# sutro-sh/sutro

Measured on AMD Instinct MI355X. Metric: output_tokens_per_sec, higher is better.
Workload: dtype bf16; 1 GPU; model=qwen-3-32b, global_batch=2048, seq_len=256, parallelism=dp1, prompt_len=128, priming=seeded

## Files before the change

### csrc/bindings.cpp

```cpp
#include <torch/extension.h>

#include <hip/hip_runtime.h>
#include <c10/hip/HIPStream.h>

#define CHECK_CUDA(x) TORCH_CHECK((x).is_cuda(), #x " must be a GPU tensor")
#define CHECK_CONTIG(x) TORCH_CHECK((x).is_contiguous(), #x " must be contiguous")
#define CHECK_BF16(x) \
  TORCH_CHECK((x).scalar_type() == at::kBFloat16, #x " must be bf16")

static hipStream_t cur_stream() {
  return c10::hip::getCurrentHIPStream().stream();
}

extern "C" {
void sutro_rmsnorm(void*, const void*, const void*, float, long, int,
                   hipStream_t);
void sutro_fused_add_rmsnorm(void*, void*, const void*, float, long, int,
                             hipStream_t);
void sutro_silu_mul(void*, const void*, long, int, hipStream_t);
void sutro_rope_and_cache(void*, void*, const void*, const long*, const long*,
                          void*, void*, const float*, int, int, int, int, int,
                          hipStream_t);
static bool is_fp8(const torch::Tensor& t) {
  return t.scalar_type() == at::kFloat8_e4m3fn;
}
void sutro_mean_pool_normalize(float*, const void*, const int*, int, int,
                               hipStream_t);
void sutro_attn_decode(void*, const void*, const void*, const void*,
                       const int*, const int*, int, int, int, int, int, int,
                       int, float, hipStream_t);
void sutro_attn_prefill(void*, const void*, const void*, const void*,
                        const int*, const int*, const int*, const int*,
                        const int*, int, int, int, int, int, int, float,
                        hipStream_t);
void sutro_mfma32_probe(float*, const void*, const void*, hipStream_t);
void sutro_gemm_tn_launch(void*, const void*, const void*, const void*, int,
                          int, long, int, int, int, int, hipStream_t);
void sutro_mfma16_probe(float*, const void*, const void*, hipStream_t);
void sutro_hd64_stage_probe(float*, float*, void*, const void*, const void*,
                            const void*, int, float, hipStream_t);
void sutro_qkv_prep(const void*, void*, void*, void*, const long*, const long*,
                    const float*, const void*, const void*, float, int, int,
                    int, int, int, int, int, hipStream_t);
void sutro_sampler_fused(const void*, int, const float*, const float*,
                         const int*, const float*, const unsigned int*, int,
                         long, int, int, int*, float*, hipStream_t);
void sutro_grouped_gemm(void*, const void*, const void*, const int*,
                        const int*, const int*, int, int, int, long, int,
                        int, hipStream_t);
void sutro_moe_combine(void*, const void*, const long*, const float*, int,
                       int, int, hipStream_t);
void sutro_logit_penalties(void*, int, const int*, const int*, const int*,
                           const int*, const int*, const float*, const float*,
                           const float*, const int*, const float*, int, int,
                           long, int, int, int, int, int, hipStream_t);
void sutro_quant_rows_fp8(void*, float*, const void*, const int*, int, long,
                          int, int, hipStream_t);
void sutro_grouped_gemm_fp8(void*, const void*, const float*, const void*,
                            const float*, const int*, const int*, const int*,
                            int, int, int, long, int, int, hipStream_t);
void sutro_quant_weight_mxfp4(void*, void*, const void*, long, int, int,
                              hipStream_t);
void sutro_grouped_gemm_mxfp4(void*, const void*, const float*, const void*,
                              const void*, const int*, const int*, const int*,
                              int, int, int, long, int, int, hipStream_t);
}

void rmsnorm(torch::Tensor out, torch::Tensor x, torch::Tensor w, double eps) {
  CHECK_CUDA(x); CHECK_CONTIG(x); CHECK_BF16(x);
  const long C = x.size(-1);
  const long rows = x.numel() / C;
  TORCH_CHECK(C % 8 == 0 && C <= 16384, "unsupported row size ", C);
  sutro_rmsnorm(out.data_ptr(), x.data_ptr(), w.data_ptr(), (float)eps, rows,
                (int)C, cur_stream());
}

void fused_add_rmsnorm(torch::Tensor x, torch::Tensor residual, torch::Tensor w,
                       double eps) {
  CHECK_CUDA(x); CHECK_CONTIG(x); CHECK_BF16(x); CHECK_CONTIG(residual);
  const long C = x.size(-1);
  const long rows = x.numel() / C;
  TORCH_CHECK(C % 8 == 0 && C <= 16384, "unsupported row size ", C);
  sutro_fused_add_rmsnorm(x.data_ptr(), residual.data_ptr(), w.data_ptr(),
                          (float)eps, rows, (int)C, cur_stream());
}

void silu_mul(torch::Tensor out, torch::Tensor x) {
  CHECK_CUDA(x); CHECK_CONTIG(x); CHECK_BF16(x);
  const long I = x.size(-1) / 2;
  const long T = x.numel() / (2 * I);
  TORCH_CHECK(I % 8 == 0, "intermediate size must be a multiple of 8");
  sutro_silu_mul(out.data_ptr(), x.data_ptr(), T, (int)I, cur_stream());
}

void rope_and_cache(torch::Tensor q, torch::Tensor k, torch::Tensor v,
                    torch::Tensor positions, torch::Tensor slot_mapping,
                    torch::Tensor k_cache, torch::Tensor v_cache,
                    torch::Tensor cos_sin) {
  CHECK_CUDA(q); CHECK_CONTIG(q); CHECK_BF16(q);
  CHECK_CONTIG(k); CHECK_CONTIG(v); CHECK_CONTIG(k_cache);
  TORCH_CHECK(cos_sin.scalar_type() == at::kFloat, "cos_sin must be f32");
  const int T = q.size(0), Hq = q.size(1), D = q.size(2);
  const int Hk = k.size(1);
  const int bs = k_cache.size(2);
  TORCH_CHECK(D % 2 == 0 && D / 2 <= 128, "unsupported head_dim ", D);
  sutro_rope_and_cache(q.data_ptr(), k.data_ptr(), v.data_ptr(),
                       positions.data_ptr<long>(), slot_mapping.data_ptr<long>(),
                       k_cache.data_ptr(), v_cache.data_ptr(),
                       cos_sin.data_ptr<float>(), T, Hq, Hk, D, bs,
                       cur_stream());
}

void mean_pool_normalize(torch::Tensor out, torch::Tensor hidden,
                         torch::Tensor qlocs) {
  CHECK_CUDA(hidden); CHECK_CONTIG(hidden); CHECK_BF16(hidden);
  const int S = out.size(0), H = hidden.size(-1);
  TORCH_CHECK(H % 8 == 0, "hidden size must be a multiple of 8");
  sutro_mean_pool_normalize(out.data_ptr<float>(), hidden.data_ptr(),
                            qlocs.data_ptr<int>(), S, H, cur_stream());
}

void paged_attention(torch::Tensor out, torch::Tensor q, torch::Tensor k_cache,
                     torch::Tensor v_cache, torch::Tensor block_tables,
                     torch::Tensor seq_lens, torch::Tensor qlocs, double scale,
                     int64_t num_decodes, torch::Tensor tile_seq,
                     torch::Tensor tile_q0, int64_t prefill_token_count) {
  CHECK_CUDA(q); CHECK_CONTIG(q); CHECK_BF16(q); CHECK_CONTIG(k_cache);
  const int Hq = q.size(1), D = q.size(2);
  const int Hk = k_cache.size(1);
  const int bs = k_cache.size(2);
  const int S = seq_lens.size(0);
  TORCH_CHECK(D == 128 || D == 64,
              "attention kernels support head_dim 64/128 (got ", D, ")");
  TORCH_CHECK(bs == 32, "attention kernels require kv_block_size 32");
  TORCH_CHECK(Hq % Hk == 0 && Hq / Hk <= 8,
              "GQA group size must divide and be <= 8");
  const int bt_stride = block_tables.size(1);
  const int n_tiles = tile_seq.numel();
  if (n_tiles > 0) {
    sutro_attn_prefill(out.data_ptr(), q.data_ptr(), k_cache.data_ptr(),
                       v_cache.data_ptr(), block_tables.data_ptr<int>(),
                       seq_lens.data_ptr<int>(), qlocs.data_ptr<int>(),
                       tile_seq.data_ptr<int>(), tile_q0.data_ptr<int>(),
                       n_tiles, bt_stride, Hq, Hk, D,
                       is_fp8(k_cache) ? 1 : 0, (float)scale, cur_stream());
  }
  if (num_decodes > 0) {
    const long dec_off = prefill_token_count;
    const int seq_offset = S - (int)num_decodes;
    const u_int16_t* qp = (const u_int16_t*)q.data_ptr();
    u_int16_t* op = (u_int16_t*)out.data_ptr();
    sutro_attn_decode(op + dec_off * Hq * D, qp + dec_off * Hq * D,
                      k_cache.data_ptr(), v_cache.data_ptr(),
                      block_tables.data_ptr<int>(), seq_lens.data_ptr<int>(),
                      bt_stride, (int)num_decodes, Hq, Hk, D,
                      is_fp8(k_cache) ? 1 : 0, seq_offset, (float)scale,
                      cur_stream());
  }
}

void qkv_prep(torch::Tensor qkv, torch::Tensor q_out, torch::Tensor k_cache,
              torch::Tensor v_cache, torch::Tensor positions,
              torch::Tensor slot_mapping, torch::Tensor cos_sin,
              c10::optional<torch::Tensor> q_norm_w,
              c10::optional<torch::Tensor> k_norm_w, double eps) {
  CHECK_CUDA(qkv); CHECK_CONTIG(qkv); CHECK_BF16(qkv);
  CHECK_CONTIG(q_out); CHECK_CONTIG(k_cache); CHECK_CONTIG(v_cache);
  const int T = qkv.size(0);
  const int Hq = q_out.size(1), D = q_out.size(2);
  const int Hk = k_cache.size(1);
  const int bs = k_cache.size(2);
  const int row_stride = qkv.size(1);
  TORCH_CHECK(row_stride == Hq * D + 2 * Hk * D, "qkv width mismatch");
  const void* qw = q_norm_w ? q_norm_w->data_ptr() : nullptr;
  const void* kw = k_norm_w ? k_norm_w->data_ptr() : nullptr;
  sutro_qkv_prep(qkv.data_ptr(), q_out.data_ptr(), k_cache.data_ptr(),
                 v_cache.data_ptr(), positions.data_ptr<long>(),
                 slot_mapping.data_ptr<long>(), cos_sin.data_ptr<float>(), qw,
                 kw, (float)eps, T, Hq, Hk, D, bs, row_stride,
                 is_fp8(k_cache) ? 1 : 0, cur_stream());
}

torch::Tensor gemm_tn(torch::Tensor x, torch::Tensor w,
                      c10::optional<torch::Tensor> res, long bm, long bn,
                      long swz, long xcd_swz) {
  CHECK_CUDA(x); CHECK_BF16(x); CHECK_CUDA(w); CHECK_BF16(w);
  TORCH_CHECK(x.is_contiguous() && w.is_contiguous(), "contiguous required");
  const long M = x.size(0), K = x.size(1), N = w.size(0);
  TORCH_CHECK(w.size(1) == K, "K mismatch");
  TORCH_CHECK(M % bm == 0 && K % 64 == 0, "shape not tile-divisible");
  auto out = torch::empty({M, N}, x.options());
  const void* rp = nullptr;
  if (res.has_value()) {
    CHECK_CUDA(*res); CHECK_BF16(*res);
    TORCH_CHECK(res->is_contiguous() && res->size(0) == M && res->size(1) == N,
                "res shape");
    rp = res->data_ptr();
  }
  sutro_gemm_tn_launch(out.data_ptr(), x.data_ptr(), w.data_ptr(), rp, (int)M,
                       (int)N, K, (int)bm, (int)bn, (int)swz, (int)xcd_swz,
                       cur_stream());
  return out;
}

torch::Tensor mfma32_probe(torch::Tensor a, torch::Tensor b) {
  CHECK_CUDA(a); CHECK_BF16(a);
  auto c = torch::zeros({32, 32}, a.options().dtype(at::kFloat));
  sutro_mfma32_probe(c.data_ptr<float>(), a.data_ptr(), b.data_ptr(),
                     cur_stream());
  return c;
}

std::vector<torch::Tensor> hd64_stage_probe(torch::Tensor q, torch::Tensor k,
                                             torch::Tensor v, long L,
                                             double scale) {
  CHECK_CUDA(q); CHECK_BF16(q);
  auto fopt = q.options().dtype(at::kFloat);
  auto vt = torch::zeros({64 * 40}, fopt);
  auto p = torch::zeros({16 * 40}, fopt);
  auto out = torch::zeros({1, 64}, q.options());
  sutro_hd64_stage_probe(vt.data_ptr<float>(), p.data_ptr<float>(),
                         out.data_ptr(), q.data_ptr(), k.data_ptr(),
                         v.data_ptr(), (int)L, (float)scale, cur_stream());
  return {vt, p, out};
}

torch::Tensor mfma16_probe(torch::Tensor a, torch::Tensor b) {
  CHECK_CUDA(a); CHECK_BF16(a);
  auto c = torch::zeros({16, 16}, a.options().dtype(at::kFloat));
  sutro_mfma16_probe(c.data_ptr<float>(), a.data_ptr(), b.data_ptr(),
                     cur_stream());
  return c;
}

void grouped_gemm(torch::Tensor out, torch::Tensor a, torch::Tensor w,
                  c10::optional<torch::Tensor> row_tok, torch::Tensor tile_off,
                  torch::Tensor counts, long max_tiles, bool gate_silu,
                  long bm) {
  TORCH_CHECK(bm == 64 || bm == 128, "bm must be 64 or 128");
  CHECK_CUDA(a); CHECK_CONTIG(a); CHECK_BF16(a);
  CHECK_CUDA(w); CHECK_CONTIG(w); CHECK_BF16(w);
  CHECK_CONTIG(out); CHECK_BF16(out);
  const long E = w.size(0), N = w.size(1), K = w.size(2);
  const long n_cols = gate_silu ? N / 2 : N;
  TORCH_CHECK(K % 64 == 0 && n_cols % 64 == 0,
              "grouped_gemm needs K, n_cols multiples of 64 (K=", K,
              ", n_cols=", n_cols, ")");
  TORCH_CHECK(a.size(1) == K, "A K mismatch");
  TORCH_CHECK(out.size(1) == n_cols, "out width mismatch");
  TORCH_CHECK(tile_off.scalar_type() == at::kInt
              && counts.scalar_type() == at::kInt, "tile_off/counts int32");
  TORCH_CHECK(tile_off.numel() == E + 1 && counts.numel() == E, "seg sizes");
  const int* rt = nullptr;
  if (row_tok.has_value()) {
    TORCH_CHECK(row_tok->scalar_type() == at::kInt, "row_tok int32");
    rt = row_tok->data_ptr<int>();
  }
  sutro_grouped_gemm(out.data_ptr(), a.data_ptr(), w.data_ptr(), rt,
                     tile_off.data_ptr<int>(), counts.data_ptr<int>(), (int)E,
                     (int)max_tiles, (int)n_cols, K, gate_silu ? 1 : 0,
                     (int)bm, cur_stream());
}

void quant_rows_fp8(torch::Tensor x, torch::Tensor out_q,
                    torch::Tensor out_scale,
                    c10::optional<torch::Tensor> row_limit, long limit_mul) {
  CHECK_CUDA(x); CHECK_CONTIG(x); CHECK_BF16(x);
  CHECK_CUDA(out_q); CHECK_CONTIG(out_q);
  CHECK_CUDA(out_scale); CHECK_CONTIG(out_scale);
  TORCH_CHECK(x.dim() == 2 && out_q.dim() == 2, "x, out_q must be 2-D");
  TORCH_CHECK(is_fp8(out_q), "out_q must be float8_e4m3fn");
  TORCH_CHECK(out_scale.scalar_type() == at::kFloat, "out_scale must be f32");
  const long R = x.size(0), K = x.size(1), Kp = out_q.size(1);
  TORCH_CHECK(K % 8 == 0 && K > 0, "K must be a positive multiple of 8");
  TORCH_CHECK(Kp == (K + 127) / 128 * 128, "out_q width must be K rounded "
              "up to 128 (K=", K, ", Kp=", Kp, ")");
  TORCH_CHECK(Kp < (1L << 31), "row too wide");
  TORCH_CHECK(out_q.size(0) >= R && out_scale.numel() >= R,
              "out_q/out_scale hold fewer rows than x");
  const int* lim = nullptr;
  if (row_limit.has_value()) {
    CHECK_CUDA(*row_limit);
    TORCH_CHECK(row_limit->scalar_type() == at::kInt
                && row_limit->numel() >= 1, "row_limit int32 scalar");
    lim = row_limit->data_ptr<int>();
  }
  sutro_quant_rows_fp8(out_q.data_ptr(), out_scale.data_ptr<float>(),
                       x.data_ptr(), lim, (int)limit_mul, R, (int)K, (int)Kp,
                       cur_stream());
}

void grouped_gemm_fp8(torch::Tensor out, torch::Tensor a_q,
                      torch::Tensor a_scale, torch::Tensor w_q,
                      torch::Tensor w_scale,
                      c10::optional<torch::Tensor> row_tok,
                      torch::Tensor tile_off, torch::Tensor counts,
                      long max_tiles, bool gate_silu, long bm) {
  TORCH_CHECK(bm == 64 || bm == 128, "bm must be 64 or 128");
  CHECK_CUDA(a_q); CHECK_CONTIG(a_q); CHECK_CUDA(w_q); CHECK_CONTIG(w_q);
  TORCH_CHECK(is_fp8(a_q) && is_fp8(w_q), "a_q, w_q must be float8_e4m3fn");
  CHECK_CUDA(a_scale); CHECK_CONTIG(a_scale);
  CHECK_CUDA(w_scale); CHECK_CONTIG(w_scale);
  TORCH_CHECK(a_scale.scalar_type() == at::kFloat
              && w_scale.scalar_type() == at::kFloat, "scales must be f32");
  CHECK_CUDA(out); CHECK_CONTIG(out); CHECK_BF16(out);
  TORCH_CHECK(w_q.dim() == 3 && a_q.dim() == 2 && out.dim() == 2, "ranks");
  const long E = w_q.size(0), N = w_q.size(1), Kp = w_q.size(2);
  const long n_cols = gate_silu ? N / 2 : N;
  TORCH_CHECK(Kp % 128 == 0 && Kp > 0 && n_cols % 64 == 0 && n_cols > 0,
              "grouped_gemm_fp8 needs Kp a multiple of 128 and n_cols of 64 "
              "(Kp=", Kp, ", n_cols=", n_cols, ")");
  TORCH_CHECK(a_q.size(1) == Kp, "A Kp mismatch");
  TORCH_CHECK(out.size(1) == n_cols, "out width mismatch");
  TORCH_CHECK(max_tiles >= 0 && out.size(0) >= max_tiles * bm,
              "out holds fewer rows than max_tiles * bm");
  TORCH_CHECK(w_scale.numel() == E * N, "w_scale must be [E, N]");
  TORCH_CHECK(tile_off.scalar_type() == at::kInt
              && counts.scalar_type() == at::kInt, "tile_off/counts int32");
  TORCH_CHECK(tile_off.numel() == E + 1 && counts.numel() == E, "seg sizes");
  const int* rt = nullptr;
  if (row_tok.has_value()) {
    TORCH_CHECK(row_tok->scalar_type() == at::kInt, "row_tok int32");
    TORCH_CHECK(row_tok->numel() >= max_tiles * bm, "row_tok too short");
    rt = row_tok->data_ptr<int>();
  } else {
    TORCH_CHECK(a_q.size(0) >= max_tiles * bm,
                "a_q holds fewer rows than max_tiles * bm");
  }
  TORCH_CHECK(!gate_silu || rt, "the gate/up stage gathers through row_tok");
  TORCH_CHECK(a_scale.numel() >= a_q.size(0), "a_scale shorter than a_q");
  sutro_grouped_gemm_fp8(out.data_ptr(), a_q.data_ptr(),
                         a_scale.data_ptr<float>(), w_q.data_ptr(),
                         w_scale.data_ptr<float>(), rt,
                         tile_off.data_ptr<int>(), counts.data_ptr<int>(),
                         (int)E, (int)max_tiles, (int)n_cols, Kp,
                         gate_silu ? 1 : 0, (int)bm, cur_stream());
}

void quant_weight_mxfp4(torch::Tensor x, torch::Tensor out_q,
                        torch::Tensor out_scale) {
  CHECK_CUDA(x); CHECK_CONTIG(x); CHECK_BF16(x);
  CHECK_CUDA(out_q); CHECK_CONTIG(out_q);
  CHECK_CUDA(out_scale); CHECK_CONTIG(out_scale);
  TORCH_CHECK(x.dim() == 2 && out_q.dim() == 2 && out_scale.dim() == 2,
              "x, out_q, out_scale must be 2-D");
  TORCH_CHECK(out_q.scalar_type() == at::kByte
              && out_scale.scalar_type() == at::kByte,
              "out_q, out_scale must be uint8");
  const long R = x.size(0), K = x.size(1);
  TORCH_CHECK(K % 8 == 0 && K > 0, "K must be a positive multiple of 8");
  const long Kp = (K + 127) / 128 * 128;
  TORCH_CHECK(Kp < (1L << 31), "row too wide");
  TORCH_CHECK(out_q.size(1) == Kp / 2 && out_scale.size(1) == Kp / 32,
              "out_q / out_scale widths must be Kp/2 and Kp/32 with Kp = K "
// ... 50 lines not shown
  TORCH_CHECK(a_scale.numel() >= a_q.size(0), "a_scale shorter than a_q");
  sutro_grouped_gemm_mxfp4(out.data_ptr(), a_q.data_ptr(),
                           a_scale.data_ptr<float>(), w_q.data_ptr(),
                           w_scale.data_ptr(), rt,
                           tile_off.data_ptr<int>(), counts.data_ptr<int>(),
                           (int)E, (int)max_tiles, (int)n_cols, Kp,
                           gate_silu ? 1 : 0, (int)bm, cur_stream());
}

void moe_combine(torch::Tensor out, torch::Tensor rows, torch::Tensor padpos,
                 torch::Tensor w) {
  CHECK_CUDA(rows); CHECK_CONTIG(rows); CHECK_BF16(rows);
  CHECK_CONTIG(out); CHECK_BF16(out);
  const long T = out.size(0), h = out.size(1), k = padpos.size(1);
  TORCH_CHECK(h % 8 == 0, "h must be a multiple of 8");
  TORCH_CHECK(padpos.scalar_type() == at::kLong, "padpos must be int64");
  TORCH_CHECK(w.scalar_type() == at::kFloat, "w must be f32");
  TORCH_CHECK(padpos.is_contiguous() && w.is_contiguous(), "contig");
  sutro_moe_combine(out.data_ptr(), rows.data_ptr(),
                    padpos.data_ptr<long>(), w.data_ptr<float>(), (int)T,
                    (int)h, (int)k, cur_stream());
}

void sampler_fused(torch::Tensor logits, torch::Tensor temps,
                   torch::Tensor topps, torch::Tensor topks, torch::Tensor us,
                   c10::optional<torch::Tensor> mask, long vl,
                   torch::Tensor out_tok, torch::Tensor out_lp) {
  CHECK_CUDA(logits); CHECK_CONTIG(logits);
  const bool f32 = logits.scalar_type() == at::kFloat;
  TORCH_CHECK(f32 || logits.scalar_type() == at::kBFloat16,
              "logits must be bf16 or f32");
  const long n = logits.size(0), v_row = logits.size(1);
  TORCH_CHECK(vl <= v_row, "vocab_limit exceeds logits row");
  TORCH_CHECK(temps.numel() >= n && topps.numel() >= n && topks.numel() >= n
              && us.numel() >= n, "param tensors too small");
  TORCH_CHECK(topks.scalar_type() == at::kInt, "topks must be int32");
  const unsigned int* mptr = nullptr;
  int w_words = 0;
  if (mask.has_value()) {
    auto& mt = mask.value();
    CHECK_CUDA(mt); CHECK_CONTIG(mt);
    TORCH_CHECK(mt.scalar_type() == at::kInt, "mask must be int32 packed");
    TORCH_CHECK(mt.size(0) == n, "mask rows mismatch");
    w_words = (int)mt.size(1);
    TORCH_CHECK((long)w_words * 32 >= vl, "mask too narrow for vocab_limit");
    mptr = (const unsigned int*)mt.data_ptr();
  }
  sutro_sampler_fused(logits.data_ptr(), f32 ? 1 : 0,
                      temps.data_ptr<float>(), topps.data_ptr<float>(),
                      topks.data_ptr<int>(), us.data_ptr<float>(), mptr,
                      (int)n, v_row, (int)vl, w_words,
                      out_tok.data_ptr<int>(), out_lp.data_ptr<float>(),
                      cur_stream());
}

void logit_penalties(torch::Tensor logits, torch::Tensor row_idx,
                     torch::Tensor hist, torch::Tensor slot,
                     torch::Tensor hist_len, torch::Tensor prompt_len,
                     torch::Tensor rep, torch::Tensor pres, torch::Tensor freq,
                     c10::optional<torch::Tensor> bias_tok,
                     c10::optional<torch::Tensor> bias_val, long vl,
                     long max_hist_len) {
  CHECK_CUDA(logits); CHECK_CONTIG(logits);
  const bool f32 = logits.scalar_type() == at::kFloat;
  TORCH_CHECK(f32 || logits.scalar_type() == at::kBFloat16,
              "logits must be bf16 or f32");
  TORCH_CHECK(logits.dim() == 2, "logits must be [n, V]");
  const long n = logits.size(0), v_row = logits.size(1);
  TORCH_CHECK(vl >= 0 && vl <= v_row, "vocab_limit exceeds logits row");
  TORCH_CHECK(v_row < (1L << 31) && n < (1L << 31), "logits too large");
  const long m = row_idx.numel();
  if (m == 0) return;
  auto chk_i32 = [&](const torch::Tensor& t, const char* name) {
    TORCH_CHECK(t.is_cuda() && t.is_contiguous()
                && t.scalar_type() == at::kInt && t.numel() == m,
                name, " must be a contiguous int32 GPU tensor of ", m);
  };
  auto chk_f32 = [&](const torch::Tensor& t, const char* name) {
    TORCH_CHECK(t.is_cuda() && t.is_contiguous()
                && t.scalar_type() == at::kFloat && t.numel() == m,
                name, " must be a contiguous f32 GPU tensor of ", m);
  };
  chk_i32(row_idx, "row_idx"); chk_i32(slot, "slot");
  chk_i32(hist_len, "hist_len"); chk_i32(prompt_len, "prompt_len");
  chk_f32(rep, "rep"); chk_f32(pres, "pres"); chk_f32(freq, "freq");
  CHECK_CUDA(hist); CHECK_CONTIG(hist);
  TORCH_CHECK(hist.scalar_type() == at::kInt && hist.dim() == 2,
              "hist must be int32 [S, Lcap]");
  const long n_slots = hist.size(0), lcap = hist.size(1);
  TORCH_CHECK(lcap < (1L << 31) && n_slots < (1L << 31), "hist too large");
  long n_bias = 0;
  const int* btp = nullptr;
  const float* bvp = nullptr;
  TORCH_CHECK(bias_tok.has_value() == bias_val.has_value(),
              "bias_tok and bias_val go together");
  if (bias_tok.has_value() && bias_tok->numel() > 0) {
    auto& bt = bias_tok.value();
    auto& bv = bias_val.value();
    CHECK_CUDA(bt); CHECK_CONTIG(bt); CHECK_CUDA(bv); CHECK_CONTIG(bv);
    TORCH_CHECK(bt.scalar_type() == at::kInt && bv.scalar_type() == at::kFloat,
                "bias_tok int32 / bias_val f32");
    TORCH_CHECK(bt.dim() == 2 && bt.size(0) == m && bv.dim() == 2
                && bv.size(0) == m && bv.size(1) == bt.size(1),
                "bias_tok/bias_val must be [m, B]");
    n_bias = bt.size(1);
    TORCH_CHECK(n_bias <= 512, "at most 512 bias entries per row");
    btp = bt.data_ptr<int>();
    bvp = bv.data_ptr<float>();
  }
  TORCH_CHECK(max_hist_len >= 0 && max_hist_len + n_bias <= 8192,
              "hist_len + bias entries above 8192: use the torch reference");
  const long need = 2 * (max_hist_len + n_bias);
  const int log2_cap = need <= 2048 ? 11 : (need <= 8192 ? 13 : 14);
  sutro_logit_penalties(logits.data_ptr(), f32 ? 1 : 0,
                        row_idx.data_ptr<int>(), hist.data_ptr<int>(),
                        slot.data_ptr<int>(), hist_len.data_ptr<int>(),
                        prompt_len.data_ptr<int>(), rep.data_ptr<float>(),
                        pres.data_ptr<float>(), freq.data_ptr<float>(), btp,
                        bvp, (int)m, (int)n, v_row, (int)vl, (int)n_slots,
                        (int)lcap, (int)n_bias, log2_cap, cur_stream());
}

PYBIND11_MODULE(TORCH_EXTENSION_NAME, m) {
  m.def("rmsnorm", &rmsnorm, "RMSNorm (bf16, CDNA4)");
  m.def("fused_add_rmsnorm", &fused_add_rmsnorm, "residual+=x; x=rmsnorm");
  m.def("silu_mul", &silu_mul, "fused SwiGLU");
  m.def("rope_and_cache", &rope_and_cache, "RoPE + paged KV write");
  m.def("qkv_prep", &qkv_prep, "fused qk-norm + RoPE + KV write + q gather");
  m.def("mean_pool_normalize", &mean_pool_normalize, "varlen mean pool + L2");
  m.def("paged_attention", &paged_attention, "paged prefill+decode attention");
  m.def("mfma32_probe", &mfma32_probe, "MFMA fragment-layout probe");
  m.def("mfma16_probe", &mfma16_probe, "16x16 MFMA fragment-layout probe");
  m.def("hd64_stage_probe", &hd64_stage_probe, "D=64 decode stage dump probe");
  m.def("moe_combine", &moe_combine, "fused MoE weighted gather-combine");
  m.def("grouped_gemm", &grouped_gemm,
        "dropless MoE grouped GEMM (padded segments, static grid)");
  m.def("quant_rows_fp8", &quant_rows_fp8,
        "bf16 rows -> e4m3 codes + f32 per-row scale (K padded to 128)");
  m.def("grouped_gemm_fp8", &grouped_gemm_fp8,
        "dropless MoE grouped GEMM, e4m3 operands on the block-scaled MFMA");
  m.def("quant_weight_mxfp4", &quant_weight_mxfp4,
        "bf16 rows -> e2m1 code pairs + e8m0 scale per 32 (K padded to 128)");
  m.def("grouped_gemm_mxfp4", &grouped_gemm_mxfp4,
        "dropless MoE grouped GEMM, e4m3 x MXFP4 on the block-scaled MFMA");
  m.def("sampler_fused", &sampler_fused,
        "fused mask+temp+topk/topp+sample+logprob (radix descent, no sort)");
  m.def("logit_penalties", &logit_penalties,
        "sparse repetition/presence/frequency penalties + logit_bias "
        "(LDS hash of the row history, in place)");
  m.def("gemm_tn", &gemm_tn, "bf16 TN GEMM (MFMA, glds dbuf)",
        py::arg("x"), py::arg("w"), py::arg("res") = c10::nullopt,
        py::arg("bm") = 256, py::arg("bn") = 256, py::arg("swz") = 2,
        py::arg("xcd_swz") = 0);
}
```

### setup.py

```python

import os

os.environ.setdefault("PYTORCH_ROCM_ARCH", "gfx950")

from setuptools import setup
from torch.utils.cpp_extension import BuildExtension, CUDAExtension

SOURCES = [
    "csrc/bindings.cpp",
    "csrc/rmsnorm.hip",
    "csrc/elementwise.hip",
    "csrc/rope_cache.hip",
    "csrc/qkv_prep.hip",
    "csrc/pool.hip",
    "csrc/attn_decode.hip",
    "csrc/attn_decode_mfma.hip",
    "csrc/attn_prefill.hip",
    "csrc/gemm_tn.hip",
    "csrc/sampler.hip",
    "csrc/grouped_gemm.hip",
    "csrc/grouped_gemm_fp8.hip",
    "csrc/grouped_gemm_mxfp4.hip",
    "csrc/logit_penalties.hip",
]

setup(
    name="sutro-amd-kernels",
    ext_modules=[
        CUDAExtension(
            name="sutro_amd._C",
            sources=SOURCES,
            extra_compile_args={
                "cxx": ["-O3"],
                "nvcc": ["-O3", "--offload-arch=gfx950"],
            },
        )
    ],
    cmdclass={"build_ext": BuildExtension},
)
```

### sutro_amd/models/qwen3.py

```python

from __future__ import annotations

import math
from typing import Optional

import torch
import torch.distributed as dist
import torch.nn as nn
import torch.nn.functional as F

from .. import ops
from ..engine.batch import ForwardBatch
from ..engine.kv_cache import PagedKVCache
from ..ops import torch_ref
from ..parallel.tp import TPContext
from .registry import ModelSpec


_MOE_WS: dict = {}


def _mark_shard(p: nn.Parameter, full_shape, dim: int, tp: TPContext,
                row_sections=None) -> None:
    p._tp_full_shape = tuple(full_shape)
    p._tp_dim = dim
    p._tp_rank = tp.rank
    p._tp_size = tp.size
    p._tp_sections = row_sections


class RMSNorm(nn.Module):
    def __init__(self, size: int, eps: float, dtype: torch.dtype):
        super().__init__()
        self.weight = nn.Parameter(torch.ones(size, dtype=dtype))
        self.eps = eps

    def forward(self, x: torch.Tensor) -> torch.Tensor:
        return ops.rmsnorm(x, self.weight, self.eps)


class Qwen3Attention(nn.Module):
    def __init__(self, spec: ModelSpec, dtype: torch.dtype, layer_idx: int,
                 tp: Optional[TPContext] = None):
        super().__init__()
        tp = tp or TPContext()
        self.tp = tp
        assert spec.num_heads % tp.size == 0, "num_heads must divide tp_size"
        assert spec.num_kv_heads % tp.size == 0 or tp.size == 1, \
            "num_kv_heads must divide tp_size"
        self.layer_idx = layer_idx
        self.num_heads = spec.num_heads // tp.size
        self.num_kv_heads = max(1, spec.num_kv_heads // tp.size)
        self.head_dim = spec.head_dim
        self.q_size = self.num_heads * self.head_dim
        self.kv_size = self.num_kv_heads * self.head_dim
        self.scale = 1.0 / math.sqrt(self.head_dim)
        h = spec.hidden_size
        qs_full = spec.num_heads * spec.head_dim
        kv_full = spec.num_kv_heads * spec.head_dim
        self.qkv_proj = nn.Linear(h, self.q_size + 2 * self.kv_size, bias=False,
                                  dtype=dtype)
        _mark_shard(self.qkv_proj.weight, (qs_full + 2 * kv_full, h), 0, tp,
                    row_sections=[(0, qs_full), (qs_full, kv_full),
                                  (qs_full + kv_full, kv_full)])
        self.o_proj = nn.Linear(self.q_size, h, bias=False, dtype=dtype)
        _mark_shard(self.o_proj.weight, (h, qs_full), 1, tp)
        self.qk_norm = spec.qk_norm
        if spec.qk_norm:
            self.q_norm = RMSNorm(self.head_dim, spec.rms_eps, dtype)
            self.k_norm = RMSNorm(self.head_dim, spec.rms_eps, dtype)

    def forward(self, x: torch.Tensor, fb: ForwardBatch, kv: PagedKVCache,
                cos_sin: torch.Tensor) -> torch.Tensor:
        T = x.shape[0]
        qkv = self.qkv_proj(x)
        q = ops.fused_qkv_prep(
            qkv, self.num_heads, self.num_kv_heads, self.head_dim,
            fb.positions, fb.slot_mapping,
            kv.k_cache[self.layer_idx], kv.v_cache[self.layer_idx], cos_sin,
            self.q_norm.weight if self.qk_norm else None,
            self.k_norm.weight if self.qk_norm else None,
            self.q_norm.eps if self.qk_norm else 1e-6,
        )
        o = ops.paged_attention(q, kv.k_cache[self.layer_idx],
                                kv.v_cache[self.layer_idx], fb.block_tables,
                                fb.seq_lens, fb.query_start_locs, self.scale,
                                fb.num_decodes_tail, fb.tile_seq, fb.tile_q0,
                                fb.prefill_token_count)
        return self.tp.all_reduce(self.o_proj(o.view(T, self.q_size)))


class Qwen3MLP(nn.Module):
    def __init__(self, hidden: int, intermediate: int, dtype: torch.dtype,
                 tp: Optional[TPContext] = None):
        super().__init__()
        tp = tp or TPContext()
        self.tp = tp
        assert intermediate % tp.size == 0
        inter_l = intermediate // tp.size
        self.gate_up_proj = nn.Linear(hidden, 2 * inter_l, bias=False, dtype=dtype)
        _mark_shard(self.gate_up_proj.weight, (2 * intermediate, hidden), 0, tp,
                    row_sections=[(0, intermediate), (intermediate, intermediate)])
        self.down_proj = nn.Linear(inter_l, hidden, bias=False, dtype=dtype)
        _mark_shard(self.down_proj.weight, (hidden, intermediate), 1, tp)

    def forward(self, x: torch.Tensor) -> torch.Tensor:
        return self.tp.all_reduce(self.down_proj(ops.silu_mul(self.gate_up_proj(x))))


class Qwen3MoE(nn.Module):

    def __init__(self, spec: ModelSpec, dtype: torch.dtype,
                 tp: Optional[TPContext] = None, ep: bool = False):
        super().__init__()
        tp = tp or TPContext()
        self.tp = tp
        self.ep = ep and tp.size > 1
        self.num_experts = spec.num_experts
        self.top_k = spec.experts_per_token
        h, m = spec.hidden_size, spec.moe_intermediate_size
        self.router = nn.Linear(h, spec.num_experts, bias=False, dtype=dtype)
        if self.ep:
            assert spec.num_experts % tp.size == 0
            e_l = spec.num_experts // tp.size
            self.experts_per_rank = e_l
            self.expert_base = tp.rank * e_l
            self.gate_up = nn.Parameter(torch.empty(e_l, 2 * m, h, dtype=dtype))
            _mark_shard(self.gate_up, (spec.num_experts, 2 * m, h), 0, tp)
            self.down = nn.Parameter(torch.empty(e_l, h, m, dtype=dtype))
            _mark_shard(self.down, (spec.num_experts, h, m), 0, tp)
        else:
            assert m % tp.size == 0
            m_l = m // tp.size
            self.experts_per_rank = spec.num_experts
            self.expert_base = 0
            self.gate_up = nn.Parameter(
                torch.empty(spec.num_experts, 2 * m_l, h, dtype=dtype))
            _mark_shard(self.gate_up, (spec.num_experts, 2 * m, h), 1, tp,
                        row_sections=[(0, m), (m, m)])
            self.down = nn.Parameter(
                torch.empty(spec.num_experts, h, m_l, dtype=dtype))
            _mark_shard(self.down, (spec.num_experts, h, m), 2, tp)

    @property
    def experts_fp8(self) -> bool:
        return self.gate_up.dtype == torch.float8_e4m3fn

    @property
    def experts_mxfp4(self) -> bool:
        return self.gate_up.dtype == torch.uint8

    @torch.no_grad()
    def quantize_experts_mxfp4(self) -> None:
        if self.experts_fp8:
            raise RuntimeError("experts are already quantised to fp8_e4m3; "
                               "mxfp4 needs the unquantised weights")
        for name in ("gate_up", "down"):
            if getattr(self, name).dtype == torch.uint8:
                continue
            w = getattr(self, name).data.contiguous()
            codes, scales = ops.quantize_weight_mxfp4(w)
            del self._parameters[name]
            del w
            self.register_buffer(name, codes)
            self.register_buffer(name + "_scales", scales)

    @torch.no_grad()
    def load_expert_mxfp4(self, name: str, codes: torch.Tensor,
                          scales: torch.Tensor) -> None:
        if self.experts_fp8:
            raise RuntimeError("experts are already quantised to fp8_e4m3")
        w = getattr(self, name)
        E, N = w.shape[:2]
        Kp = (w.shape[2] * 2 if w.dtype == torch.uint8
              else torch_ref.fp8_padded_k(w.shape[2]))
        if (codes.dtype != torch.uint8 or scales.dtype != torch.uint8
                or tuple(codes.shape) != (E, N, Kp // 2)
                or tuple(scales.shape) != (E, N, Kp // 32)):
            raise ValueError(
                f"MXFP4 pair for {name} must be uint8 {(E, N, Kp // 2)} / "
                f"{(E, N, Kp // 32)} (the local shard), got "
                f"{codes.dtype} {tuple(codes.shape)} / "
                f"{scales.dtype} {tuple(scales.shape)}")
        dev = w.device
        self._parameters.pop(name, None)
        self._buffers.pop(name, None)
        self._buffers.pop(name + "_scales", None)
        del w
        self.register_buffer(name, codes.to(dev).contiguous())
        self.register_buffer(name + "_scales", scales.to(dev).contiguous())

    def _expert_k(self, name: str) -> int:
        w = getattr(self, name)
        return w.shape[2] * 2 if self.experts_mxfp4 else w.shape[2]

    @torch.no_grad()
    def quantize_experts_fp8(self) -> None:
        if self.experts_fp8:
            return
        if self.experts_mxfp4:
            raise RuntimeError("experts are already quantised to mxfp4; "
                               "fp8_e4m3 needs the unquantised weights")
        for name in ("gate_up", "down"):
            w = getattr(self, name).data.contiguous()
            E, N, K = w.shape
            Kp = torch_ref.fp8_padded_k(K)
            w_q = torch.empty(E, N, Kp, dtype=torch.float8_e4m3fn,
                              device=w.device)
            scale = torch.empty(E, N, dtype=torch.float32, device=w.device)
            ops.quantize_rows_fp8(w.view(E * N, K), w_q.view(E * N, Kp),
                                  scale.view(-1))
            del self._parameters[name]
            del w
            self.register_buffer(name, w_q)
            self.register_buffer(name + "_scale", scale)

    def _expert_mlp(self, seg: torch.Tensor, e: int) -> torch.Tensor:
        mx = self.experts_mxfp4
        if not (self.experts_fp8 or mx):
            act = ops.silu_mul(seg @ self.gate_up[e].T)
            return act @ self.down[e].T
        n = seg.shape[0]
        m = self.gate_up.shape[1] // 2
        dev = seg.device

        def quant(rows):
            q = torch.empty(n, torch_ref.fp8_padded_k(rows.shape[1]),
                            dtype=torch.float8_e4m3fn, device=dev)
            s = torch.empty(n, dtype=torch.float32, device=dev)
            return ops.quantize_rows_fp8(rows.contiguous(), q, s)

        x_q, x_s = quant(seg)
        if mx:
            y = torch_ref.mxfp4_linear(x_q, x_s, self.gate_up[e],
                                       self.gate_up_scales[e])
        else:
            y = torch_ref.fp8_linear(x_q, x_s, self.gate_up[e],
                                     self.gate_up_scale[e])
        act = (F.silu(y[:, :m]) * y[:, m:]).to(seg.dtype)
        a_q, a_s = quant(act)
        if mx:
            return torch_ref.mxfp4_linear(a_q, a_s, self.down[e],
                                          self.down_scales[e]).to(seg.dtype)
        return torch_ref.fp8_linear(a_q, a_s, self.down[e],
                                    self.down_scale[e]).to(seg.dtype)

    def forward(self, x: torch.Tensor) -> torch.Tensor:
        if x.is_cuda:
            if (self._PREFILL_BLASLT_MIN
                    and not (self.experts_fp8 or self.experts_mxfp4)
                    and x.shape[0] >= self._PREFILL_BLASLT_MIN
                    and not torch.cuda.is_current_stream_capturing()):
                return self.tp.all_reduce(self._forward_prefill_blaslt(x))
            return self.tp.all_reduce(self._forward_grouped(x))
        return self.tp.all_reduce(self._forward_loop(x))

    def _forward_loop(self, x: torch.Tensor) -> torch.Tensor:
        T, h = x.shape
        weights, idx = torch_ref.topk_softmax_router(self.router(x), self.top_k)
        flat_expert = idx.reshape(-1)
# ... 351 lines not shown
```

### sutro_amd/ops/__init__.py

```python

from __future__ import annotations

import os
from typing import Optional

import torch

from . import torch_ref

_C = None
_C_ERR: Optional[str] = None
try:
    from sutro_amd import _C as _C
except Exception as e:
    _C_ERR = f"{type(e).__name__}: {e}"


def hip_available() -> bool:
    return _C is not None


def _require_hip():
    if _C is None:
        raise RuntimeError(
            "sutro_amd HIP extension (_C) is not built but a GPU tensor was passed. "
            "Build it with `python setup.py build_ext --inplace` "
            f"(import error: {_C_ERR})"
        )
    return _C


_FORCE_REF = os.environ.get("SUTRO_AMD_FORCE_TORCH_REF", "0") == "1"


def _use_hip(t: torch.Tensor) -> bool:
    return t.is_cuda and not _FORCE_REF


def rmsnorm(x: torch.Tensor, weight: torch.Tensor, eps: float) -> torch.Tensor:
    if _use_hip(x):
        out = torch.empty_like(x)
        _require_hip().rmsnorm(out, x, weight, eps)
        return out
    return torch_ref.rmsnorm(x, weight, eps)


def fused_add_rmsnorm(x, residual, weight, eps: float):
    if _use_hip(x):
        _require_hip().fused_add_rmsnorm(x, residual, weight, eps)
        return x, residual
    return torch_ref.fused_add_rmsnorm(x, residual, weight, eps)


def silu_mul(x: torch.Tensor) -> torch.Tensor:
    if _use_hip(x):
        T, two_i = x.shape
        out = torch.empty((T, two_i // 2), dtype=x.dtype, device=x.device)
        _require_hip().silu_mul(out, x)
        return out
    return torch_ref.silu_mul(x)


def fused_qkv_prep(
    qkv: torch.Tensor,
    num_heads: int, num_kv_heads: int, head_dim: int,
    positions: torch.Tensor, slot_mapping: torch.Tensor,
    k_cache: torch.Tensor, v_cache: torch.Tensor,
    cos_sin: torch.Tensor,
    q_norm_w: Optional[torch.Tensor] = None,
    k_norm_w: Optional[torch.Tensor] = None,
    eps: float = 1e-6,
) -> torch.Tensor:
    T = qkv.shape[0]
    if _use_hip(qkv):
        q_out = torch.empty((T, num_heads, head_dim), dtype=qkv.dtype,
                            device=qkv.device)
        _require_hip().qkv_prep(qkv, q_out, k_cache, v_cache, positions,
                                slot_mapping, cos_sin, q_norm_w, k_norm_w, eps)
        return q_out
    q_size = num_heads * head_dim
    kv_size = num_kv_heads * head_dim
    q, k, v = qkv.split([q_size, kv_size, kv_size], dim=-1)
    q = q.reshape(T, num_heads, head_dim).contiguous()
    k = k.reshape(T, num_kv_heads, head_dim).contiguous()
    v = v.reshape(T, num_kv_heads, head_dim).contiguous()
    if q_norm_w is not None:
        q = torch_ref.rmsnorm(q, q_norm_w, eps)
    if k_norm_w is not None:
        k = torch_ref.rmsnorm(k, k_norm_w, eps)
    q, k = torch_ref.apply_rope(q, k, positions, cos_sin)
    torch_ref.write_kv_cache(k, v, k_cache, v_cache, slot_mapping)
    return q


def rope_and_cache(
    q: torch.Tensor, k: torch.Tensor, v: torch.Tensor,
    positions: torch.Tensor, slot_mapping: torch.Tensor,
    k_cache: torch.Tensor, v_cache: torch.Tensor,
    cos_sin: torch.Tensor,
) -> torch.Tensor:
    if _use_hip(q):
        _require_hip().rope_and_cache(q, k, v, positions, slot_mapping,
                                      k_cache, v_cache, cos_sin)
        return q
    q, k = torch_ref.apply_rope(q, k, positions, cos_sin)
    torch_ref.write_kv_cache(k, v, k_cache, v_cache, slot_mapping)
    return q


_EMPTY_I32: Optional[torch.Tensor] = None


def paged_attention(
    q: torch.Tensor, k_cache: torch.Tensor, v_cache: torch.Tensor,
    block_tables: torch.Tensor, seq_lens: torch.Tensor,
    query_start_locs: torch.Tensor, scale: float,
    num_decodes_tail: int = 0,
    tile_seq: Optional[torch.Tensor] = None,
    tile_q0: Optional[torch.Tensor] = None,
    prefill_token_count: int = 0,
) -> torch.Tensor:
    if _use_hip(q):
        out = torch.empty_like(q)
        if tile_seq is None:
            tile_seq = torch.empty(0, dtype=torch.int32, device=q.device)
            tile_q0 = tile_seq
        _require_hip().paged_attention(out, q, k_cache, v_cache, block_tables,
                                       seq_lens, query_start_locs, scale,
                                       num_decodes_tail, tile_seq, tile_q0,
                                       prefill_token_count)
        return out
    return torch_ref.paged_attention(q, k_cache, v_cache, block_tables,
                                     seq_lens, query_start_locs, scale)


def mean_pool_normalize(hidden: torch.Tensor, query_start_locs: torch.Tensor) -> torch.Tensor:
    if _use_hip(hidden):
        S = query_start_locs.numel() - 1
        out = torch.empty((S, hidden.shape[-1]), dtype=torch.float32, device=hidden.device)
        _require_hip().mean_pool_normalize(out, hidden, query_start_locs)
        return out
    return torch_ref.mean_pool_normalize(hidden, query_start_locs)


def sampler_fused(logits, temps, top_ps, top_ks, u, packed_mask, vocab_limit,
                  out_tok, out_lp):
    _require_hip().sampler_fused(logits, temps, top_ps, top_ks, u,
                                 packed_mask, vocab_limit, out_tok, out_lp)


def grouped_gemm(out, a, w, row_tok, tile_off, counts, max_tiles, gate_silu,
                 bm=64):
    if _use_hip(a):
        _require_hip().grouped_gemm(out, a, w, row_tok, tile_off, counts,
                                    max_tiles, gate_silu, bm)
        return out
    return torch_ref.grouped_gemm(out, a, w, row_tok, tile_off, counts,
                                  max_tiles, gate_silu, bm)


def quantize_rows_fp8(x, out_q, out_scale, row_limit=None, limit_mul=1):
    if _use_hip(x):
        _require_hip().quant_rows_fp8(x, out_q, out_scale, row_limit,
                                      limit_mul)
        return out_q, out_scale
    return torch_ref.quantize_rows_fp8(x, out_q, out_scale, row_limit,
                                       limit_mul)


def grouped_gemm_fp8(out, a_q, a_scale, w_q, w_scale, row_tok, tile_off,
                     counts, max_tiles, gate_silu, bm=64):
    if _use_hip(a_q):
        _require_hip().grouped_gemm_fp8(out, a_q, a_scale, w_q, w_scale,
                                        row_tok, tile_off, counts, max_tiles,
                                        gate_silu, bm)
        return out
    return torch_ref.grouped_gemm_fp8(out, a_q, a_scale, w_q, w_scale,
                                      row_tok, tile_off, counts, max_tiles,
                                      gate_silu, bm)


def quantize_weight_mxfp4(w):
    if _use_hip(w):
        *lead, K = w.shape
        Kp = torch_ref.fp8_padded_k(K)
        w2 = w.contiguous().view(-1, K)
        codes = torch.empty(w2.shape[0], Kp // 2, dtype=torch.uint8,
                            device=w.device)
        scales = torch.empty(w2.shape[0], Kp // 32, dtype=torch.uint8,
                             device=w.device)
        _require_hip().quant_weight_mxfp4(w2, codes, scales)
        return codes.view(*lead, Kp // 2), scales.view(*lead, Kp // 32)
    return torch_ref.quantize_weight_mxfp4(w)


def grouped_gemm_mxfp4(out, a_q, a_scale, codes, scales, row_tok, tile_off,
                       counts, max_tiles, gate_silu, bm=64):
    if _use_hip(a_q):
        _require_hip().grouped_gemm_mxfp4(out, a_q, a_scale, codes, scales,
                                          row_tok, tile_off, counts,
                                          max_tiles, gate_silu, bm)
        return out
    return torch_ref.grouped_gemm_mxfp4(out, a_q, a_scale, codes, scales,
                                        row_tok, tile_off, counts, max_tiles,
                                        gate_silu, bm)


def moe_combine(out, rows, padpos, w):
    if _use_hip(rows):
        _require_hip().moe_combine(out, rows, padpos, w)
        return out
    contrib = rows[padpos].float()
    out.copy_((contrib * w.unsqueeze(-1)).sum(dim=1).to(out.dtype))
# ... 28 lines not shown
```

Baseline: 7182 tokens/s.

## Fuse SwiGLU into a new pipelined bf16 gate_up GEMM kernel

```diff
diff --git a/csrc/bindings.cpp b/csrc/bindings.cpp
--- a/csrc/bindings.cpp
+++ b/csrc/bindings.cpp
@@ -36,6 +36,8 @@
 void sutro_mfma32_probe(float*, const void*, const void*, hipStream_t);
 void sutro_gemm_tn_launch(void*, const void*, const void*, const void*, int,
                           int, long, int, int, int, int, hipStream_t);
+int sutro_gemm_tn_pipe_launch(void*, const void*, const void*, const void*,
+                              int, int, long, int, int, int, hipStream_t);
 void sutro_mfma16_probe(float*, const void*, const void*, hipStream_t);
 void sutro_hd64_stage_probe(float*, float*, void*, const void*, const void*,
                             const void*, int, float, hipStream_t);
@@ -200,6 +202,53 @@
   sutro_gemm_tn_launch(out.data_ptr(), x.data_ptr(), w.data_ptr(), rp, (int)M,
                        (int)N, K, (int)bm, (int)bn, (int)swz, (int)xcd_swz,
                        cur_stream());
+  return out;
+}
+
+torch::Tensor gemm_tn_pipelined(torch::Tensor x, torch::Tensor w,
+                                c10::optional<torch::Tensor> res, long swz,
+                                long xcd_swz) {
+  CHECK_CUDA(x); CHECK_BF16(x); CHECK_CUDA(w); CHECK_BF16(w);
+  TORCH_CHECK(x.dim() == 2 && w.dim() == 2, "x and w must be 2-d");
+  TORCH_CHECK(x.is_contiguous() && w.is_contiguous(), "contiguous required");
+  const long M = x.size(0), K = x.size(1), N = w.size(0);
+  TORCH_CHECK(w.size(1) == K, "K mismatch");
+  TORCH_CHECK(M >= 1 && N >= 1 && K >= 64 && K % 64 == 0,
+              "shape not tile-divisible");
+  TORCH_CHECK(M < (1L << 31) && N < (1L << 31), "M/N too large");
+  TORCH_CHECK(swz >= 0 && swz <= 2, "swz must be 0, 1 or 2");
+  auto out = torch::empty({M, N}, x.options());
+  const void* rp = nullptr;
+  if (res.has_value()) {
+    CHECK_CUDA(*res); CHECK_BF16(*res);
+    TORCH_CHECK(res->is_contiguous() && res->dim() == 2 &&
+                res->size(0) == M && res->size(1) == N, "res shape");
+    rp = res->data_ptr();
+  }
+  const int e = sutro_gemm_tn_pipe_launch(
+      out.data_ptr(), x.data_ptr(), w.data_ptr(), rp, (int)M, (int)N, K,
+      rp ? 1 : 0, (int)swz, (int)xcd_swz, cur_stream());
+  TORCH_CHECK(e == 0, "gemm_tn_pipelined launch setup failed: ", e);
+  return out;
+}
+
+torch::Tensor gemm_gate_up_silu(torch::Tensor x, torch::Tensor w, long swz,
+                                long xcd_swz) {
+  CHECK_CUDA(x); CHECK_BF16(x); CHECK_CUDA(w); CHECK_BF16(w);
+  TORCH_CHECK(x.dim() == 2 && w.dim() == 2, "x and w must be 2-d");
+  TORCH_CHECK(x.is_contiguous() && w.is_contiguous(), "contiguous required");
+  const long M = x.size(0), K = x.size(1), N = w.size(0);
+  TORCH_CHECK(w.size(1) == K, "K mismatch");
+  TORCH_CHECK(M >= 1 && K >= 64 && K % 64 == 0, "shape not tile-divisible");
+  TORCH_CHECK(N >= 256 && N % 256 == 0,
+              "gate_up rows must be 2*I with I % 128 == 0");
+  TORCH_CHECK(M < (1L << 31) && N < (1L << 31), "M/N too large");
+  TORCH_CHECK(swz >= 0 && swz <= 2, "swz must be 0, 1 or 2");
+  auto out = torch::empty({M, N / 2}, x.options());
+  const int e = sutro_gemm_tn_pipe_launch(
+      out.data_ptr(), x.data_ptr(), w.data_ptr(), nullptr, (int)M, (int)N, K,
+      2, (int)swz, (int)xcd_swz, cur_stream());
+  TORCH_CHECK(e == 0, "gemm_gate_up_silu launch setup failed: ", e);
   return out;
 }
 
@@ -556,4 +605,12 @@
         py::arg("x"), py::arg("w"), py::arg("res") = c10::nullopt,
         py::arg("bm") = 256, py::arg("bn") = 256, py::arg("swz") = 2,
         py::arg("xcd_swz") = 0);
-}
+  m.def("gemm_tn_pipelined", &gemm_tn_pipelined,
+        "bf16 TN GEMM (MFMA, 8-phase glds pipeline, any M/N)",
+        py::arg("x"), py::arg("w"), py::arg("res") = c10::nullopt,
+        py::arg("swz") = 2, py::arg("xcd_swz") = 1);
+  m.def("gemm_gate_up_silu", &gemm_gate_up_silu,
+        "SwiGLU fused into the pipelined gate_up GEMM",
+        py::arg("x"), py::arg("w"), py::arg("swz") = 2,
+        py::arg("xcd_swz") = 1);
+}
diff --git a/csrc/gemm_tn_pipe.hip b/csrc/gemm_tn_pipe.hip
--- /dev/null
+++ b/csrc/gemm_tn_pipe.hip
@@ -0,0 +1,289 @@
+#include "common.h"
+
+typedef s16x8 bf16x8;
+
+namespace {
+
+__device__ __forceinline__ f32x4 mfma16(bf16x8 a, bf16x8 b, f32x4 c) {
+  return __builtin_amdgcn_mfma_f32_16x16x32_bf16(a, b, c, 0, 0, 0);
+}
+
+__device__ __forceinline__ void glds16(const char* g, char* lds) {
+  __builtin_amdgcn_global_load_lds(
+      (const __attribute__((address_space(1))) u32*)g,
+      (__attribute__((address_space(3))) u32*)lds, 16, 0, 0);
+}
+
+template <int SWZ>
+__device__ __forceinline__ u32 swz(u32 byte) {
+  if (SWZ == 1) return byte ^ (((byte >> 9) & 1u) << 5);
+  if (SWZ == 2) return byte ^ (((byte >> 8) & 7u) << 4);
+  return byte;
+}
+
+constexpr int HT = 16384;
+constexpr int KTILE_B = 65536;
+constexpr int SLOT_B0 = 0, SLOT_A0 = 1, SLOT_B1 = 2, SLOT_A1 = 3;
+
+struct Src {
+  const char* p[2];
+};
+
+template <int SWZ>
+__device__ __forceinline__ Src make_src(const u16* base, long row0,
+                                        long rows_valid, long Kb, int wave,
+                                        int lane) {
+  Src s;
+#pragma unroll
+  for (int j = 0; j < 2; ++j) {
+    const u32 b = (u32)(wave * 2 + j) * 1024u + (u32)lane * 16u;
+    const u32 lb = swz<SWZ>(b);
+    long row = (long)(lb >> 7);
+    row = row < rows_valid ? row : rows_valid - 1;
+    s.p[j] = (const char*)base + (row0 + row) * Kb + (lb & 127u);
+  }
+  return s;
+}
+
+__device__ __forceinline__ void stage_half(char* slot_wave, const Src& s,
+                                           long koff) {
+  glds16(s.p[0] + koff, slot_wave);
+  glds16(s.p[1] + koff, slot_wave + 1024);
+}
+
+__device__ __forceinline__ bf16x8 lds_frag(const char* smem, u32 off) {
+  return *(const bf16x8*)(smem + off);
+}
+
+}
+
+template <int EPI, int SWZ>
+__global__ __launch_bounds__(512) void gemm_tn_pipe_kernel(
+    u16* __restrict__ out, const u16* __restrict__ x,
+    const u16* __restrict__ w, const u16* __restrict__ res, int M, int N,
+    long K, int xcd_swz) {
+  extern __shared__ __attribute__((aligned(1024))) char smem[];
+
+  const int lane = threadIdx.x & 63;
+  const int wave = __builtin_amdgcn_readfirstlane(threadIdx.x >> 6);
+  const int wm = wave >> 2;
+  const int wn = wave & 3;
+
+  int bid = blockIdx.x;
+  if (xcd_swz) {
+    const int nwg = gridDim.x;
+    const int q = nwg >> 3, r = nwg & 7;
+    const int xcd = bid & 7, seq = bid >> 3;
+    bid = (xcd < r ? xcd * (q + 1) : r * (q + 1) + (xcd - r) * q) + seq;
+  }
+  const int MT = (M + 255) >> 8;
+  const int m0 = (bid % MT) * 256;
+  const int I = N >> 1;
+  const int nt = bid / MT;
+  const int nb0 = (EPI == 2) ? nt * 128 : nt * 256;
+  const int nb1 = (EPI == 2) ? I + nt * 128 : nt * 256 + 128;
+  const int nlim = (EPI == 2) ? I : N;
+
+  const long Kb = K * 2;
+  const long a0v = min(128, M - m0);
+  const long a1v = max(1, min(128, M - m0 - 128));
+  const long b0v = min(128, nlim - nb0);
+  const long b1v = (EPI == 2) ? 128 : max(1, min(128, N - nb1));
+  const long a1r = (M - m0 - 128 >= 1) ? m0 + 128 : m0 + a0v - 1;
+  const long b1r = (EPI == 2 || N - nb1 >= 1) ? nb1 : nb0 + b0v - 1;
+  const Src sB0 = make_src<SWZ>(w, nb0, b0v, Kb, wave, lane);
+  const Src sA0 = make_src<SWZ>(x, m0, a0v, Kb, wave, lane);
+  const Src sB1 = make_src<SWZ>(w, b1r, b1v, Kb, wave, lane);
+  const Src sA1 = make_src<SWZ>(x, a1r, a1v, Kb, wave, lane);
+
+  char* const sw = smem + wave * 2048;
+
+  u32 aoff[2], boff[2];
+#pragma unroll
+  for (int kk = 0; kk < 2; ++kk) {
+    const u32 kc = (u32)(kk * 4 + (lane >> 4)) * 16u;
+    aoff[kk] = swz<SWZ>((u32)(wm * 64 + (lane & 15)) * 128u + kc);
+    boff[kk] = swz<SWZ>((u32)(wn * 32 + (lane & 15)) * 128u + kc);
+  }
+
+  f32x4 acc[2][2][4][2];
+#pragma unroll
+  for (int a = 0; a < 2; ++a)
+#pragma unroll
+    for (int b = 0; b < 2; ++b)
+#pragma unroll
+      for (int i = 0; i < 4; ++i)
+#pragma unroll
+        for (int j = 0; j < 2; ++j) acc[a][b][i][j] = f32x4{0.f, 0.f, 0.f, 0.f};
+
+  const int KT = (int)(K >> 6);
+  const int klast = KT - 1;
+
+  {
+    const long k1 = (long)min(1, klast) * 128;
+    stage_half(sw + SLOT_B0 * HT, sB0, 0);
+    stage_half(sw + SLOT_A0 * HT, sA0, 0);
+    stage_half(sw + SLOT_B1 * HT, sB1, 0);
+    stage_half(sw + SLOT_A1 * HT, sA1, 0);
+    stage_half(sw + KTILE_B + SLOT_B0 * HT, sB0, k1);
+    stage_half(sw + KTILE_B + SLOT_A0 * HT, sA0, k1);
+    stage_half(sw + KTILE_B + SLOT_B1 * HT, sB1, k1);
+    asm volatile("s_waitcnt vmcnt(6)" ::: "memory");
+    __builtin_amdgcn_s_barrier();
+    if (wm == 1) __builtin_amdgcn_s_barrier();
+  }
+
+  bf16x8 fa[4][2], fb0[2][2], fb1[2][2];
+
+#define PHASE_SYNC_MFMA(A_, B_, FB_)                                     \
+  __builtin_amdgcn_sched_barrier(0);                                     \
+  __builtin_amdgcn_s_barrier();                                          \
+  asm volatile("s_waitcnt lgkmcnt(0)" ::: "memory");                     \
+  __builtin_amdgcn_sched_barrier(0);                                     \
+  __builtin_amdgcn_s_setprio(1);                                         \
+  _Pragma("unroll") for (int kk = 0; kk < 2; ++kk)                       \
+  _Pragma("unroll") for (int i = 0; i < 4; ++i)                          \
+  _Pragma("unroll") for (int j = 0; j < 2; ++j)                          \
+      acc[A_][B_][i][j] = mfma16(fa[i][kk], FB_[j][kk], acc[A_][B_][i][j]); \
+  __builtin_amdgcn_s_setprio(0);                                         \
+  __builtin_amdgcn_sched_barrier(0);                                     \
+  __builtin_amdgcn_s_barrier();                                          \
+  __builtin_amdgcn_sched_barrier(0);
+
+#define KTILE(P)                                                         \
+  {                                                                      \
+    const char* cur = smem + (P) * KTILE_B;                              \
+    char* nxt = sw + ((P) ^ 1) * KTILE_B;                                \
+    char* own = sw + (P) * KTILE_B;                                      \
+                                                                \
+    _Pragma("unroll") for (int j = 0; j < 2; ++j)                        \
+    _Pragma("unroll") for (int kk = 0; kk < 2; ++kk)                     \
+        fb0[j][kk] = lds_frag(cur + SLOT_B0 * HT + j * 2048, boff[kk]);  \
+    __builtin_amdgcn_sched_barrier(0);                                   \
+    _Pragma("unroll") for (int i = 0; i < 4; ++i)                        \
+    _Pragma("unroll") for (int kk = 0; kk < 2; ++kk)                     \
+        fa[i][kk] = lds_frag(cur + SLOT_A0 * HT + i * 2048, aoff[kk]);   \
+    __builtin_amdgcn_sched_barrier(0);                                   \
+    stage_half(nxt + SLOT_A1 * HT, sA1, kn1);                            \
+    __builtin_amdgcn_sched_barrier(0);                                   \
+    asm volatile("s_waitcnt lgkmcnt(8)" ::: "memory");                   \
+    PHASE_SYNC_MFMA(0, 0, fb0)                                           \
+                                                                \
+    _Pragma("unroll") for (int j = 0; j < 2; ++j)                        \
+    _Pragma("unroll") for (int kk = 0; kk < 2; ++kk)                     \
+        fb1[j][kk] = lds_frag(cur + SLOT_B1 * HT + j * 2048, boff[kk]);  \
+    __builtin_amdgcn_sched_barrier(0);                                   \
+    stage_half(own + SLOT_B0 * HT, sB0, kn2);                            \
+    PHASE_SYNC_MFMA(0, 1, fb1)                                           \
+                                                                \
+    _Pragma("unroll") for (int i = 0; i < 4; ++i)                        \
+    _Pragma("unroll") for (int kk = 0; kk < 2; ++kk)                     \
+        fa[i][kk] = lds_frag(cur + SLOT_A1 * HT + i * 2048, aoff[kk]);   \
+    __builtin_amdgcn_sched_barrier(0);                                   \
+    stage_half(own + SLOT_A0 * HT, sA0, kn2);                            \
+    PHASE_SYNC_MFMA(1, 0, fb0)                                           \
+                                                                \
+    stage_half(own + SLOT_B1 * HT, sB1, kn2);                            \
+    __builtin_amdgcn_sched_barrier(0);                                   \
+    asm volatile("s_waitcnt vmcnt(6)" ::: "memory");                     \
+    PHASE_SYNC_MFMA(1, 1, fb1)                                           \
+  }
+
+  for (int t = 0; t < KT; t += 2) {
+    {
+      const long kn1 = (long)min(t + 1, klast) * 128;
+      const long kn2 = (long)min(t + 2, klast) * 128;
+      KTILE(0)
+    }
+    if (t + 1 < KT) {
+      const long kn1 = (long)min(t + 2, klast) * 128;
+      const long kn2 = (long)min(t + 3, klast) * 128;
+      KTILE(1)
+    }
+  }
+#undef KTILE
+#undef PHASE_SYNC_MFMA
+
+  asm volatile("s_waitcnt vmcnt(0)" ::: "memory");
+  if (wm == 0) __builtin_amdgcn_s_barrier();
+
+  const int drow = (lane >> 4) * 4;
+  const int dcol = lane & 15;
+  if (EPI == 2) {
+#pragma unroll
+    for (int a = 0; a < 2; ++a)
+#pragma unroll
+      for (int i = 0; i < 4; ++i)
+#pragma unroll
+        for (int j = 0; j < 2; ++j) {
+          const int gn = nb0 + wn * 32 + j * 16 + dcol;
+          const int gm = m0 + a * 128 + wm * 64 + i * 16 + drow;
+#pragma unroll
+          for (int r = 0; r < 4; ++r) {
+            if (gm + r >= M) continue;
+            const float gf = bf2f(f2bf(acc[a][0][i][j][r]));
+            const float uf = bf2f(f2bf(acc[a][1][i][j][r]));
+            const float s = gf / (1.f + __expf(-gf));
+            out[(long)(gm + r) * I + gn] = f2bf(s * uf);
+          }
+        }
+  } else {
+#pragma unroll
+    for (int a = 0; a < 2; ++a)
+#pragma unroll
+      for (int b = 0; b < 2; ++b)
+#pragma unroll
+        for (int i = 0; i < 4; ++i)
+#pragma unroll
+          for (int j = 0; j < 2; ++j) {
+            const int gn = nb0 + b * 128 + wn * 32 + j * 16 + dcol;
+            if (gn >= N) continue;
+            const int gm = m0 + a * 128 + wm * 64 + i * 16 + drow;
+#pragma unroll
+            for (int r = 0; r < 4; ++r) {
+              if (gm + r >= M) continue;
+              const long o = (long)(gm + r) * N + gn;
+              float v = acc[a][b][i][j][r];
+              if (EPI == 1) v += bf2f(res[o]);
+              out[o] = f2bf(v);
+            }
+          }
+  }
+}
+
+extern "C" int sutro_gemm_tn_pipe_launch(void* out, const void* x,
+                                         const void* w, const void* res,
+                                         int M, int N, long K, int epi,
+                                         int swz_mode, int xcd_swz,
+                                         hipStream_t stream) {
+  constexpr int LDS_BYTES = 2 * KTILE_B;
+  const int mt = (M + 255) / 256;
+  const int ntl = (epi == 2) ? (N / 2) / 128 : (N + 255) / 256;
+  dim3 grid(mt * ntl), block(512);
+  constexpr int MAX_DEV = 64;
+  static bool attr_set[3][3][MAX_DEV];
+  int dev = 0;
+  const int ed = (int)hipGetDevice(&dev);
+  if (ed != 0) return ed;
+#define LAUNCH_1(EPI, SWZ)                                                   \
+  if (epi == EPI && swz_mode == SWZ) {                                       \
+    if (dev < 0 || dev >= MAX_DEV || !attr_set[EPI][SWZ][dev]) {             \
+      const int e = (int)hipFuncSetAttribute(                                \
+          (const void*)gemm_tn_pipe_kernel<EPI, SWZ>,                        \
+          hipFuncAttributeMaxDynamicSharedMemorySize, LDS_BYTES);            \
+      if (e != 0) return e;                                                  \
+      if (dev >= 0 && dev < MAX_DEV) attr_set[EPI][SWZ][dev] = true;         \
+    }                                                                        \
+    gemm_tn_pipe_kernel<EPI, SWZ><<<grid, block, LDS_BYTES, stream>>>(       \
+        (u16*)out, (const u16*)x, (const u16*)w, (const u16*)res, M, N, K,   \
+        xcd_swz);                                                            \
+    return 0;                                                                \
+  }
+#define LAUNCH(EPI) LAUNCH_1(EPI, 0) LAUNCH_1(EPI, 1) LAUNCH_1(EPI, 2)
+  LAUNCH(0)
+  LAUNCH(1)
+  LAUNCH(2)
+#undef LAUNCH
+#undef LAUNCH_1
+  return -1;
+}
diff --git a/setup.py b/setup.py
--- a/setup.py
+++ b/setup.py
@@ -17,6 +17,7 @@
     "csrc/attn_decode_mfma.hip",
     "csrc/attn_prefill.hip",
     "csrc/gemm_tn.hip",
+    "csrc/gemm_tn_pipe.hip",
     "csrc/sampler.hip",
     "csrc/grouped_gemm.hip",
     "csrc/grouped_gemm_fp8.hip",
diff --git a/sutro_amd/models/qwen3.py b/sutro_amd/models/qwen3.py
--- a/sutro_amd/models/qwen3.py
+++ b/sutro_amd/models/qwen3.py
@@ -105,7 +105,8 @@
         _mark_shard(self.down_proj.weight, (hidden, intermediate), 1, tp)
 
     def forward(self, x: torch.Tensor) -> torch.Tensor:
-        return self.tp.all_reduce(self.down_proj(ops.silu_mul(self.gate_up_proj(x))))
+        act = ops.gate_up_silu(x, self.gate_up_proj.weight)
+        return self.tp.all_reduce(self.down_proj(act))
 
 
 class Qwen3MoE(nn.Module):
diff --git a/sutro_amd/ops/__init__.py b/sutro_amd/ops/__init__.py
--- a/sutro_amd/ops/__init__.py
+++ b/sutro_amd/ops/__init__.py
@@ -59,6 +59,41 @@
         _require_hip().silu_mul(out, x)
         return out
     return torch_ref.silu_mul(x)
+
+
+GATE_UP_FUSED_RULE: dict = {
+    (5120, 51200): (1152, frozenset({1536, 1664, 1792})),
+}
+
+_GATE_UP_FORCE: Optional[bool] = {"1": True, "0": False}.get(
+    os.environ.get("SUTRO_GATE_UP_FUSED", ""))
+
+
+def set_gate_up_fused(mode: Optional[bool]) -> None:
+    global _GATE_UP_FORCE
+    _GATE_UP_FORCE = mode
+
+
+def gate_up_silu_qualifies(x: torch.Tensor, weight: torch.Tensor) -> bool:
+    return (x.dim() == 2 and weight.dim() == 2 and x.shape[0] >= 1
+            and x.dtype == torch.bfloat16 and weight.dtype == torch.bfloat16
+            and x.is_contiguous() and weight.is_contiguous()
+            and x.shape[1] == weight.shape[1] and x.shape[1] % 64 == 0
+            and weight.shape[0] >= 256 and weight.shape[0] % 256 == 0)
+
+
+def gate_up_silu(x: torch.Tensor, weight: torch.Tensor) -> torch.Tensor:
+    if _use_hip(x) and gate_up_silu_qualifies(x, weight):
+        if _GATE_UP_FORCE is None:
+            min_m, held_back = GATE_UP_FUSED_RULE.get(
+                (x.shape[1], weight.shape[0]), (None, ()))
+            fused = (min_m is not None and x.shape[0] >= min_m
+                     and x.shape[0] not in held_back)
+        else:
+            fused = _GATE_UP_FORCE
+        if fused:
+            return _require_hip().gemm_gate_up_silu(x, weight)
+    return silu_mul(torch.nn.functional.linear(x, weight))
 
 
 def fused_qkv_prep(
```

Result: faster. 7338 tokens/s, median of 6 (+2.2%).
